# nvagus/mnexp

Measured on NVIDIA B200. Metric: lstur_train_impressions_per_sec, higher is better.
Workload: dtype f16

## Files before the change

### mnexp_b200/csrc/attn.cu

```cuda
#include <cuda_fp16.h>

#include <stdlib.h>

#include "common.cuh"

namespace lstur {

constexpr int ATT_THREADS = 128;
constexpr int ATT_MAX_L = 256;

__global__ void __launch_bounds__(ATT_THREADS)
attn_pool_fwd_kernel(int N, int L, int F, float* __restrict__ C, long long title_stride,
                     const int* __restrict__ tok, const float* __restrict__ ka, const float* __restrict__ ba,
                     float* __restrict__ p, long long ldp, float* __restrict__ a_out, float* __restrict__ w_out,
                     uint32_t drop_thr, float inv_keep, uint32_t seed) {
  __shared__ float sa[ATT_MAX_L], se[ATT_MAX_L];
  const int n = blockIdx.x, tid = threadIdx.x, warp = tid >> 5, lane = tid & 31;
  float* Cn = C + (long long)n * title_stride;
  const float bias = ba[0];
  for (int t = warp; t < L; t += ATT_THREADS / 32) {
    const int tk = tok[(long long)n * L + t];
    float dot = 0.f;
    int any = 0;
    const uint64_t base = ((uint64_t)n * L + t) * (uint64_t)F;
    for (int f = lane; f < F; f += 32) {
      float v = tk != 0 ? Cn[(long long)t * F + f] : 0.f;
      any |= (v != 0.f);
      if (drop_thr) v = (rng_u32(seed, base + f) >> 8) >= drop_thr ? v * inv_keep : 0.f;
      Cn[(long long)t * F + f] = v;
      dot = fmaf(v, ka[f], dot);
    }
    any = warp_or(any);
    dot = warp_sum(dot);
    if (lane == 0) {
      float a = tanhf(dot + bias);
      sa[t] = a;
      se[t] = any ? expf(a) : 0.f;
    }
  }
  __syncthreads();
  float S = 0.f;
  for (int t = 0; t < L; ++t) S += se[t];
  const float invS = 1.f / (S + 1e-7f);
  for (int t = tid; t < L; t += ATT_THREADS) {
    if (a_out) a_out[(long long)n * L + t] = sa[t];
    if (w_out) w_out[(long long)n * L + t] = se[t] * invS;
  }
  for (int f = tid; f < F; f += ATT_THREADS) {
    float acc = 0.f;
    for (int t = 0; t < L; ++t) acc = fmaf(se[t] * invS, Cn[(long long)t * F + f], acc);
    p[(long long)n * ldp + f] = acc;
  }
}

__device__ __forceinline__ float ldc(const float* p, long long i) { return p[i]; }
__device__ __forceinline__ float ldc(const __nv_bfloat16* p, long long i) { return __bfloat162float(p[i]); }
__device__ __forceinline__ float ldc(const __half* p, long long i) { return __half2float(p[i]); }

__device__ __forceinline__ void store_dpre_img(void* img, int out_mode, int ngh, int Fh, int n, int t, int f, float v) {
  const int h = f >= Fh ? 1 : 0, fl = f - h * Fh;
  const long long byte = (long long)n * ((long long)2 * ngh * 4096) + (long long)(h * ngh + (fl >> 6)) * 4096 + t * 128 +
                         ((((fl & 63) >> 3) ^ (t & 7)) << 4) + (fl & 7) * 2;
  if (out_mode == 2) *reinterpret_cast<__half*>((char*)img + byte) = __float2half_rn(fminf(fmaxf(v, -65504.f), 65504.f));
  else *reinterpret_cast<__nv_bfloat16*>((char*)img + byte) = __float2bfloat16_rn(v);
}

template <int FPT, typename CT, int OUT>
__global__ void __launch_bounds__(ATT_THREADS)
attn_pool_bwd_kernel(int N, int L, int Lrows, int F, const CT* __restrict__ Cd, long long title_stride,
                     const float* __restrict__ a_in, const float* __restrict__ w_in, const float* __restrict__ dp,
                     long long lddp, const float* __restrict__ ka, float* __restrict__ dPre,
                     long long dpre_title_stride, float inv_keep, float* __restrict__ partials) {
  __shared__ float sdw[ATT_MAX_L], sdz[ATT_MAX_L], sw[ATT_MAX_L];
  const int tid = threadIdx.x, warp = tid >> 5, lane = tid & 31;
  float dka[FPT], dbc[FPT], dba = 0.f;
#pragma unroll
  for (int i = 0; i < FPT; ++i) dka[i] = dbc[i] = 0.f;
  for (int n = blockIdx.x; n < N; n += gridDim.x) {
    const CT* Cn = Cd + (long long)n * title_stride;
    const float* dpn = dp + (long long)n * lddp;
    float* dPn = dPre + (long long)n * dpre_title_stride;
    for (int t = warp; t < L; t += ATT_THREADS / 32) {
      float dot = 0.f;
      for (int f = lane; f < F; f += 32) dot = fmaf(ldc(Cn, (long long)t * F + f), dpn[f], dot);
      dot = warp_sum(dot);
      if (lane == 0) {
        sdw[t] = dot;
        sw[t] = w_in[(long long)n * L + t];
      }
    }
    __syncthreads();
    float q = 0.f;
    for (int t = 0; t < L; ++t) q = fmaf(sdw[t], sw[t], q);
    for (int t = tid; t < L; t += ATT_THREADS) {
      float a = a_in[(long long)n * L + t];
      sdz[t] = (sdw[t] - q) * sw[t] * (1.f - a * a);
    }
    __syncthreads();
#pragma unroll
    for (int i = 0; i < FPT; ++i) {
      int f = tid + i * ATT_THREADS;
      if (f < F) {
        const float dpf = dpn[f], kaf = ka[f];
        for (int t = 0; t < L; ++t) {
          float c = ldc(Cn, (long long)t * F + f);
          float g = fmaf(sw[t], dpf, sdz[t] * kaf);
          float dpre = c > 0.f ? g * inv_keep : 0.f;
          if (OUT == 0) dPn[(long long)t * F + f] = dpre;
          else store_dpre_img(dPre, OUT, ((F >> 1) + 63) >> 6, F >> 1, n, t, f, dpre);
          dka[i] = fmaf(sdz[t], c, dka[i]);
          dbc[i] += dpre;
        }
        for (int t = L; t < Lrows; ++t) {
          if (OUT == 0) dPn[(long long)t * F + f] = 0.f;
          else store_dpre_img(dPre, OUT, ((F >> 1) + 63) >> 6, F >> 1, n, t, f, 0.f);
        }
      }
    }
    if (tid == 0)
      for (int t = 0; t < L; ++t) dba += sdz[t];
    __syncthreads();
  }
  float* out = partials + (long long)blockIdx.x * (2 * F + 1);
#pragma unroll
  for (int i = 0; i < FPT; ++i) {
    int f = tid + i * ATT_THREADS;
    if (f < F) {
      out[f] = dka[i];
      out[F + f] = dbc[i];
    }
  }
  if (tid == 0) out[2 * F] = dba;
}

__global__ void colsum_stage1_kernel(long long rows, int cols, const float* __restrict__ in, long long ld,
                                     int rows_per_chunk, float* __restrict__ partial) {
  int c = blockIdx.x * blockDim.x + threadIdx.x;
  if (c >= cols) return;
  long long r0 = (long long)blockIdx.y * rows_per_chunk, r1 = min(rows, r0 + rows_per_chunk);
  float s0 = 0.f, s1 = 0.f, s2 = 0.f, s3 = 0.f;
  long long r = r0;
  for (; r + 3 < r1; r += 4) {
    s0 += in[r * ld + c];
    s1 += in[(r + 1) * ld + c];
    s2 += in[(r + 2) * ld + c];
    s3 += in[(r + 3) * ld + c];
  }
  for (; r < r1; ++r) s0 += in[r * ld + c];
  partial[(long long)blockIdx.y * cols + c] = (s0 + s1) + (s2 + s3);
}
__global__ void colsum_stage2_kernel(int chunks, int cols, const float* __restrict__ partial, float* __restrict__ out,
                                     int accumulate) {
  __shared__ float sm[8][32];
  const int lane = threadIdx.x & 31, part = threadIdx.x >> 5;
  const int c = blockIdx.x * 32 + lane;
  float s = 0.f;
  if (c < cols)
    for (int k = part; k < chunks; k += 8) s += partial[(long long)k * cols + c];
  sm[part][lane] = s;
  __syncthreads();
  if (part != 0 || c >= cols) return;
  float t = 0.f;
#pragma unroll
  for (int q = 0; q < 8; ++q) t += sm[q][lane];
  out[c] = accumulate ? out[c] + t : t;
}

template <typename CT>
__device__ __forceinline__ void unpack8(const uint4& u, float* v);
template <>
__device__ __forceinline__ void unpack8<__half>(const uint4& u, float* v) {
  const __half2* h = reinterpret_cast<const __half2*>(&u);
#pragma unroll
  for (int i = 0; i < 4; ++i) { float2 f = __half22float2(h[i]); v[2 * i] = f.x; v[2 * i + 1] = f.y; }
}
template <>
__device__ __forceinline__ void unpack8<__nv_bfloat16>(const uint4& u, float* v) {
  const __nv_bfloat162* h = reinterpret_cast<const __nv_bfloat162*>(&u);
#pragma unroll
  for (int i = 0; i < 4; ++i) { float2 f = __bfloat1622float2(h[i]); v[2 * i] = f.x; v[2 * i + 1] = f.y; }
}
template <typename CT>
__device__ __forceinline__ uint4 pack8(const float* v);
template <>
__device__ __forceinline__ uint4 pack8<__half>(const float* v) {
  uint4 u;
  __half2* h = reinterpret_cast<__half2*>(&u);
#pragma unroll
  for (int i = 0; i < 4; ++i) {
    uint32_t w;
    asm("cvt.rn.satfinite.f16x2.f32 %0, %1, %2;" : "=r"(w) : "f"(v[2 * i + 1]), "f"(v[2 * i]));
    reinterpret_cast<uint32_t*>(&u)[i] = w;
  }
  (void)h;
  return u;
}
template <>
__device__ __forceinline__ uint4 pack8<__nv_bfloat16>(const float* v) {
  uint4 u;
  __nv_bfloat162* h = reinterpret_cast<__nv_bfloat162*>(&u);
#pragma unroll
  for (int i = 0; i < 4; ++i) h[i] = __floats2bfloat162_rn(v[2 * i], v[2 * i + 1]);
  return u;
}

constexpr int IMG_THREADS = 256;
template <typename CT, int SLOT>
__global__ void __launch_bounds__(IMG_THREADS)
attn_bwd_img_kernel(int N, int L, int F, const CT* __restrict__ Cd, const float* __restrict__ a_in,
                    const float* __restrict__ w_in, const float* __restrict__ dp, long long lddp,
                    const float* __restrict__ ka, uint8_t* __restrict__ img, float inv_keep, float img_scale,
                    float* __restrict__ partials, int nbuf, const int* __restrict__ n_dev,
                    const int* __restrict__ title_idx) {
  if (n_dev) N = min(N, __ldg(n_dev));
  extern __shared__ __align__(16) uint8_t att_smem[];
  const int nchunk = F >> 3;
  const size_t buf_bytes = (size_t)SLOT * nchunk * 16;
  float* sdp = reinterpret_cast<float*>(att_smem + nbuf * buf_bytes);
  float* ska = sdp + F;
  float* sred = reinterpret_cast<float*>(att_smem);
  __shared__ float sdw[SLOT], sdz[SLOT], sw[SLOT];
  __shared__ __align__(8) unsigned long long s_bar[2];
  const int tid = threadIdx.x, warp = tid >> 5, lane = tid & 31;
  const int c = tid & 63, tg = tid >> 6;
  const bool c_ok = c < nchunk;
  const int Fh = F >> 1, ngh = (Fh + 63) >> 6;
  constexpr int GROUP_BYTES = SLOT * 128;
  const long long blk_bytes = (long long)2 * ngh * GROUP_BYTES;
  const int pad_pieces = ((((Fh + 31) >> 5) << 5) - Fh) >> 3;
  const uint32_t title_bytes = (uint32_t)L * F * sizeof(CT);
  const uint32_t bar0 = (uint32_t)__cvta_generic_to_shared(&s_bar[0]);
  const uint32_t buf0 = (uint32_t)__cvta_generic_to_shared(att_smem);
  auto fetch_title = [&](int n, int b) {
    asm volatile("mbarrier.arrive.expect_tx.shared::cta.b64 _, [%0], %1;" ::"r"(bar0 + 8 * b), "r"(title_bytes) : "memory");
    asm volatile("cp.async.bulk.shared::cluster.global.mbarrier::complete_tx::bytes [%0], [%1], %2, [%3];" ::"r"(
                     buf0 + (uint32_t)(b * buf_bytes)),
                 "l"(Cd + (long long)n * L * F), "r"(title_bytes), "r"(bar0 + 8 * b)
                 : "memory");
  };
  if (tid == 0) {
    asm volatile("mbarrier.init.shared::cta.b64 [%0], 1;" ::"r"(bar0) : "memory");
    asm volatile("mbarrier.init.shared::cta.b64 [%0], 1;" ::"r"(bar0 + 8) : "memory");
    asm volatile("fence.mbarrier_init.release.cluster;" ::: "memory");
  }
  for (int f = tid; f < F; f += IMG_THREADS) ska[f] = ka[f];
  __syncthreads();
  float dka[8], dbc[8], dba = 0.f;
#pragma unroll
  for (int i = 0; i < 8; ++i) dka[i] = dbc[i] = 0.f;
  constexpr int DPR = 2;
  float ndp[DPR], nw = 0.f, na = 0.f;
  auto prefetch_small = [&](int n) {
    const int no = (title_idx && n < N) ? __ldg(title_idx + n) : n;
#pragma unroll
    for (int i = 0; i < DPR; ++i) {
      const int f = tid + i * IMG_THREADS;
      ndp[i] = (n < N && f < F) ? dp[(long long)no * lddp + f] : 0.f;
    }
    nw = (n < N && tid < L) ? w_in[(long long)n * L + tid] : 0.f;
    na = (n < N && tid < L) ? a_in[(long long)n * L + tid] : 0.f;
  };
  if (blockIdx.x < N) {
    if (tid == 0) fetch_title(blockIdx.x, 0);
    prefetch_small(blockIdx.x);
  }
  uint32_t phase[2] = {0, 0};
  int it = 0;
  for (int n = blockIdx.x; n < N; n += gridDim.x, ++it) {
    const int b = nbuf == 2 ? (it & 1) : 0;
    const uint4* sC = reinterpret_cast<const uint4*>(att_smem + b * buf_bytes);
    __syncthreads();
    const int n_next = n + gridDim.x;
    if (nbuf == 2) {
      if (tid == 0 && n_next < N) fetch_title(n_next, b ^ 1);
    } else if (it > 0) {
      if (tid == 0) fetch_title(n, 0);
    }
#pragma unroll
    for (int i = 0; i < DPR; ++i) {
      const int f = tid + i * IMG_THREADS;
      if (f < F) sdp[f] = ndp[i];
    }
    if (tid < L) sw[tid] = nw;
    const float a_cur = na;
    prefetch_small(n_next);
    {
      uint32_t done = 0;
      while (!done) {
        asm volatile(
            "{\n\t.reg .pred p;\n\t"
            "mbarrier.try_wait.parity.shared::cta.b64 p, [%1], %2;\n\t"
            "selp.u32 %0, 1, 0, p;\n\t}"
            : "=r"(done)
            : "r"(bar0 + 8 * b), "r"(phase[b])
            : "memory");
      }
      phase[b] ^= 1;
    }
    __syncthreads();
    {
      float dpa[2][8];
#pragma unroll
      for (int k = 0; k < 2; ++k) {
        const int cc = lane + 32 * k;
        const float4 lo = cc < nchunk ? *reinterpret_cast<const float4*>(sdp + cc * 8) : make_float4(0.f, 0.f, 0.f, 0.f);
        const float4 hi = cc < nchunk ? *reinterpret_cast<const float4*>(sdp + cc * 8 + 4) : make_float4(0.f, 0.f, 0.f, 0.f);
        dpa[k][0] = lo.x; dpa[k][1] = lo.y; dpa[k][2] = lo.z; dpa[k][3] = lo.w;
        dpa[k][4] = hi.x; dpa[k][5] = hi.y; dpa[k][6] = hi.z; dpa[k][7] = hi.w;
      }
#pragma unroll
      for (int tt = 0; tt < SLOT / 8; ++tt) {
// ... 282 lines not shown
```

### mnexp_b200/csrc/gather.cu

```cuda
#include "common.cuh"

namespace lstur {

__global__ void token_gather_kernel(int N, int L, int n_docs, const int* __restrict__ doc_tokens,
                                    const int* __restrict__ doc_ids, int* __restrict__ tokens) {
  int warp = (blockIdx.x * blockDim.x + threadIdx.x) >> 5, lane = threadIdx.x & 31;
  if (warp >= N) return;
  int d = doc_ids[warp];
  d = (d < 0 || d >= n_docs) ? 0 : d;
  const int* src = doc_tokens + (long long)d * L;
  int* dst = tokens + (long long)warp * L;
  for (int l = lane; l < L; l += 32) dst[l] = __ldg(src + l);
}

__global__ void embed_gather_pad_kernel(int N, int L, int E, int V, int KS, const float* __restrict__ word_emb,
                                        const int* __restrict__ tok, float* __restrict__ Xp, uint32_t drop_thr,
                                        float inv_keep, uint32_t seed, int Ep) {
  long long row = ((long long)blockIdx.x * blockDim.x + threadIdx.x) >> 5;
  int lane = threadIdx.x & 31;
  const int Lp = L + KS - 1;
  if (row >= (long long)N * Lp) return;
  int n = (int)(row / Lp), t = (int)(row % Lp) - (KS - 1) / 2;
  float* dst = Xp + row * E;
  if (t < 0 || t >= L) {
    for (int e = lane; e < E; e += 32) dst[e] = 0.f;
    return;
  }
  int id = tok[(long long)n * L + t];
  id = (id < 0 || id >= V) ? 0 : id;
  const float* src = word_emb + (long long)id * E;
  const uint64_t base = ((uint64_t)n * L + t) * (uint64_t)E;
  if (Ep > 0) {
    const uint64_t pbase = ((uint64_t)n * L + t) * (uint64_t)Ep;
    for (int e = lane; e < E; e += 32) {
      float v = __ldg(src + e);
      uint32_t h = rng_u32(seed, (pbase + e) >> 1);
      uint32_t h16 = (e & 1) ? (h >> 16) : (h & 0xffffu);
      dst[e] = h16 >= drop_thr ? v * inv_keep : 0.f;
    }
    return;
  }
  if ((E & 3) == 0) {
    for (int e = lane * 4; e < E; e += 128) {
      float4 v = __ldg((const float4*)(src + e));
      if (drop_thr) {
        v.x = (rng_u32(seed, base + e + 0) >> 8) >= drop_thr ? v.x * inv_keep : 0.f;
        v.y = (rng_u32(seed, base + e + 1) >> 8) >= drop_thr ? v.y * inv_keep : 0.f;
        v.z = (rng_u32(seed, base + e + 2) >> 8) >= drop_thr ? v.z * inv_keep : 0.f;
        v.w = (rng_u32(seed, base + e + 3) >> 8) >= drop_thr ? v.w * inv_keep : 0.f;
      }
      *(float4*)(dst + e) = v;
    }
  } else {
    for (int e = lane; e < E; e += 32) {
      float v = __ldg(src + e);
      if (drop_thr) v = (rng_u32(seed, base + e) >> 8) >= drop_thr ? v * inv_keep : 0.f;
      dst[e] = v;
    }
  }
}

__global__ void hist_mask_apply_kernel(int rows, int L, int D, const int* __restrict__ tok, float* __restrict__ H,
                                       long long ldh, float* __restrict__ hm_out, float* __restrict__ gm_out) {
  int warp = (blockIdx.x * blockDim.x + threadIdx.x) >> 5, lane = threadIdx.x & 31;
  if (warp >= rows) return;
  int nz = 1;
  if (tok) {
    nz = 0;
    for (int l = lane; l < L; l += 32) nz |= (tok[(long long)warp * L + l] != 0);
    nz = warp_or(nz);
  }
  float* h = H + (long long)warp * ldh;
  int any = 0;
  for (int d = lane; d < D; d += 32) {
    float v = nz ? h[d] : 0.f;
    h[d] = v;
    any |= (v != 0.f);
  }
  any = warp_or(any);
  if (lane == 0) {
    if (hm_out) hm_out[warp] = (tok ? nz : any) ? 1.f : 0.f;
    gm_out[warp] = any ? 1.f : 0.f;
  }
}

__global__ void row_gather_kernel(int B, int D, int n_rows, const float* __restrict__ table,
                                  const int* __restrict__ ids, const float* __restrict__ scale,
                                  float* __restrict__ out, long long ldo) {
  int warp = (blockIdx.x * blockDim.x + threadIdx.x) >> 5, lane = threadIdx.x & 31;
  if (warp >= B) return;
  int id = ids[warp];
  id = (id < 0 || id >= n_rows) ? 0 : id;
  float s = scale ? scale[warp] : 1.f;
  for (int d = lane; d < D; d += 32) out[(long long)warp * ldo + d] = __ldg(table + (long long)id * D + d) * s;
}


__global__ void vert_concat_kernel(int n, int D, int col0, int dv, int ds, int n_docs, int n_vert, int n_sub,
                                   const int* __restrict__ doc_ids, const int* __restrict__ doc_vert,
                                   const int* __restrict__ doc_subvert, const float* __restrict__ vert_emb,
                                   const float* __restrict__ subvert_emb, float* __restrict__ docv,
                                   int* __restrict__ tv, int* __restrict__ ts) {
  int warp = (blockIdx.x * blockDim.x + threadIdx.x) >> 5, lane = threadIdx.x & 31;
  if (warp >= n) return;
  int d = warp;
  if (doc_ids) {
    d = doc_ids[warp];
    d = (d < 0 || d >= n_docs) ? 0 : d;
  }
  int v = dv ? doc_vert[d] : 0, sv = ds ? doc_subvert[d] : 0;
  v = (v < 0 || v >= n_vert) ? 0 : v;
  sv = (sv < 0 || sv >= n_sub) ? 0 : sv;
  float* row = docv + (long long)warp * D + col0;
  for (int j = lane; j < dv; j += 32) row[j] = vert_emb[(long long)v * dv + j];
  for (int j = lane; j < ds; j += 32) row[dv + j] = subvert_emb[(long long)sv * ds + j];
  if (lane == 0) {
    if (tv) tv[warp] = v;
    if (ts) ts[warp] = sv;
  }
}

constexpr int STG_CHUNKS = 64;
__global__ void small_table_grad1_kernel(int n, int D, int col0, int dim, const int* __restrict__ ids,
                                         const float* __restrict__ dd, float* __restrict__ partial) {
  const int r = blockIdx.x, k = blockIdx.y, n_rows = gridDim.x;
  const int per = (n + STG_CHUNKS - 1) / STG_CHUNKS;
  const int beg = k * per, end = min(n, beg + per);
  float acc = 0.f;
  const int j = threadIdx.x;
  for (int i = beg; i < end; ++i)
    if (ids[i] == r && j < dim) acc += dd[(long long)i * D + col0 + j];
  if (j < dim) partial[((long long)k * n_rows + r) * dim + j] = acc;
}
__global__ void small_table_grad2_kernel(int n_rows, int dim, const float* __restrict__ partial, float* __restrict__ out) {
  const int i = blockIdx.x * blockDim.x + threadIdx.x;
  if (i >= n_rows * dim) return;
  float acc = 0.f;
  for (int k = 0; k < STG_CHUNKS; ++k) acc += partial[(long long)k * n_rows * dim + i];
  out[i] = acc;
}
__global__ void scale_rows_kernel(int B, int D, const float* __restrict__ scale, float* __restrict__ x, long long ld) {
  const long long i = (long long)blockIdx.x * blockDim.x + threadIdx.x;
  if (i >= (long long)B * D) return;
  const int b = (int)(i / D), d = (int)(i % D);
  x[(long long)b * ld + d] *= scale[b];
}


__global__ void assemble_batch_kernel(int B, int W, int K, const int* __restrict__ sample_click, const int* __restrict__ idx,
                                      const int* __restrict__ click_user, const int* __restrict__ stream_off,
                                      const int* __restrict__ stream_docs, const int* __restrict__ neg_off,
                                      const int* __restrict__ neg_docs, uint32_t seed, int* __restrict__ user_out,
                                      int* __restrict__ hist_out, int* __restrict__ cand_out) {
  const int T = W + 1 + K;
  const long long i = (long long)blockIdx.x * blockDim.x + threadIdx.x;
  if (i >= (long long)B * T) return;
  const int b = (int)(i / T), e = (int)(i % T);
  const int c = sample_click[idx[b]];
  const int u = click_user[c];
  const int off = stream_off[u];
  if (e < W) {
    const int j = c - W + e;
    hist_out[(long long)b * W + e] = j >= off ? stream_docs[j] : 0;
    if (e == 0) user_out[b] = u;
  } else if (e == W) {
    cand_out[(long long)b * (1 + K)] = stream_docs[c];
  } else {
    const int k = e - W - 1;
    const int n0 = neg_off[c], n = neg_off[c + 1] - n0;
    const uint32_t r = rng_u32(seed, (uint64_t)b * K + k);
    cand_out[(long long)b * (1 + K) + 1 + k] = n > 0 ? neg_docs[n0 + (int)(r % (uint32_t)n)] : 0;
  }
}

__global__ void title_live_kernel(int N, int L, const int* __restrict__ tok, int* __restrict__ flags) {
  int warp = (int)(((long long)blockIdx.x * blockDim.x + threadIdx.x) >> 5), lane = threadIdx.x & 31;
  if (warp >= N) return;
  int nz = 0;
  for (int l = lane; l < L; l += 32) nz |= (tok[(long long)warp * L + l] != 0);
  nz = warp_or(nz);
  if (lane == 0) flags[warp] = nz ? 1 : 0;
}
__global__ void __launch_bounds__(1024) title_rank_kernel(int N, const int* __restrict__ flags, int* __restrict__ local_rank,
                                                          int* __restrict__ block_tot) {
  __shared__ int wsum[32];
  const int n = blockIdx.x * 1024 + threadIdx.x, lane = threadIdx.x & 31, warp = threadIdx.x >> 5;
  const int f = (n < N && flags[n]) ? 1 : 0;
  const unsigned bal = __ballot_sync(0xffffffffu, f);
  if (lane == 0) wsum[warp] = __popc(bal);
  __syncthreads();
  if (warp == 0) {
    int v = wsum[lane];
#pragma unroll
    for (int o = 1; o < 32; o <<= 1) {
      const int u = __shfl_up_sync(0xffffffffu, v, o);
      if (lane >= o) v += u;
    }
    wsum[lane] = v;
  }
  __syncthreads();
  if (n < N) local_rank[n] = (warp ? wsum[warp - 1] : 0) + __popc(bal & ((1u << lane) - 1u));
  if (threadIdx.x == 0) block_tot[blockIdx.x] = wsum[31];
}
__global__ void title_compact_kernel(int N, int L, const int* __restrict__ tok, const int* __restrict__ flags,
                                     const int* __restrict__ local_rank, const int* __restrict__ block_tot, int n_blocks,
                                     int* __restrict__ live_idx, int* __restrict__ n_live, int* __restrict__ tok_c) {
  int warp = (int)(((long long)blockIdx.x * blockDim.x + threadIdx.x) >> 5), lane = threadIdx.x & 31;
  if (warp >= N) return;
  const int blk = warp >> 10;
  int before = 0;
  for (int b = lane; b < n_blocks; b += 32) before += (b < blk || warp == N - 1) ? block_tot[b] : 0;
  before = __reduce_add_sync(0xffffffffu, before);
  if (warp == N - 1) {
    if (lane == 0) *n_live = before;
    before = 0;
    for (int b = lane; b < blk; b += 32) before += block_tot[b];
    before = __reduce_add_sync(0xffffffffu, before);
  }
  if (!flags[warp]) return;
  const int ci = before + local_rank[warp];
  if (lane == 0) live_idx[ci] = warp;
  for (int l = lane; l < L; l += 32) tok_c[(long long)ci * L + l] = tok[(long long)warp * L + l];
}

__global__ void mask_live_kernel(int N, const int* __restrict__ v, int* __restrict__ flags) {
  const int n = blockIdx.x * blockDim.x + threadIdx.x;
  if (n < N) flags[n] = v[n] != 0 ? 1 : 0;
}
__global__ void __launch_bounds__(1024) mask_compact_kernel(int N, const int* __restrict__ v, const int* __restrict__ flags,
                                                            const int* __restrict__ local_rank,
// ... 163 lines not shown
```

### mnexp_b200/csrc/gemm_tc.cu

```cuda
#include <stdlib.h>

#include "tc_common.cuh"

namespace lstur {
namespace tc {

constexpr int G_KBLK = 64;
constexpr int G_STAGES = 4;
constexpr int G_A_BYTES = TILE_M * 128;
constexpr int G_B_BYTES = 256 * 128;
constexpr int G_STAGE_BYTES = G_A_BYTES + G_B_BYTES;
constexpr int G_STAGE_BYTES_S3 = 2 * (G_A_BYTES + G_B_BYTES);
constexpr int G_THREADS = 416;
constexpr int G_PRODUCERS = 256;

struct GemmParams {
  int M, N, K;
  const float* A; long long lda;
  const float* B; long long ldb;
  float* C; long long ldc;
  const float* bias;
  int flags, ntile, k_per_split, vec_ok;
  int tiles_m, tiles_n, splits;
  float* partial;
// ... 167 lines not shown
              const uint64_t ad = TA ? make_desc_mn128(a_addr + kk * 2048, 8192) : make_desc_k128(a_addr + kk * 32);
              const uint64_t bd = TB ? make_desc_k128(b_addr + kk * 32) : make_desc_mn128(b_addr + kk * 2048, 8192);
              umma_bf16(tacc, ad, bd, idesc, accum);
              accum = 1;
              if (SPLIT) {
                const uint64_t al = TA ? make_desc_mn128(a_addr + LO_OFF + kk * 2048, 8192) : make_desc_k128(a_addr + LO_OFF + kk * 32);
                const uint64_t bl = TB ? make_desc_k128(b_addr + LO_OFF + kk * 32) : make_desc_mn128(b_addr + LO_OFF + kk * 2048, 8192);
                umma_bf16(tacc, al, bd, idesc, 1);
                umma_bf16(tacc, ad, bl, idesc, 1);
              }
            }
            umma_commit(bar_empty + 8 * s);
          }
          accum = 1;
          __syncwarp();
          if (++s == STAGES) { s = 0; ph ^= 1; }
        }
        if (leader) umma_commit(bar_t_full + 8 * acc);
        __syncwarp();
        pht[acc] ^= 1;
        acc ^= 1;
      }
    }
  } else if (warp >= 1 && warp < 9) {
    const int pt = threadIdx.x - 32;
    int s = 0;
    uint32_t ph = 0;
    constexpr int BATCH = 6;
    for (int t = blockIdx.x; t < n_tiles; t += gridDim.x) {
      const Tile x = tile_of(t);
      const int m0 = x.m0, n0 = x.n0, nt = x.nt, kend = x.kend;
      const int bgroups = (x.nmma + 63) >> 6;
      const bool img = p.bimg != nullptr;
      const int nb_pieces = img ? 0 : (TB ? x.nmma * 8 : bgroups * 512);
      const uint32_t b_tile_bytes = (uint32_t)(TB ? x.nmma * 128 : bgroups * 8192);
      int arow[4];
#pragma unroll
      for (int idx = 0; idx < 4; ++idx) {
        const int r = m0 + ((pt + idx * G_PRODUCERS) >> 3);
        arow[idx] = r < Meff ? (p.midx ? __ldg(p.midx + r) : r) : p.M;
      }
      for (int kb = 0; kb < x.nkb; ++kb) {
        const int k0 = x.kbeg + kb * G_KBLK;
        const uint32_t a_addr = smem_base + s * STAGE_BYTES, b_addr = a_addr + G_A_BYTES;
        auto piece_load = [&](int idx, float* v) {
          if (idx < 4) {
            const int i = pt + idx * G_PRODUCERS, c = i & 7, r = i >> 3;
            if (!TA) load_raw(p.A, p.lda, arow[idx], p.M, k0 + 8 * c, kend, p.vec_ok, v);
            else load_raw(p.A, p.lda, k0 + (r & 63), kend, m0 + (r >> 6) * 64 + 8 * c, p.M, p.vec_ok, v);
          } else {
            const int i = pt + (idx - 4) * G_PRODUCERS, c = i & 7, r = i >> 3;
            if (i < nb_pieces) {
              if (TB) load_raw(p.B, p.ldb, n0 + r, n0 + nt, k0 + 8 * c, kend, p.vec_ok, v);
              else load_raw(p.B, p.ldb, k0 + (r & 63), kend, n0 + (r >> 6) * 64 + 8 * c, n0 + nt, p.vec_ok, v);
            }
          }
        };
        auto piece_store = [&](int idx, const float* v) {
          uint4 lo;
          if (idx < 4) {
            const int i = pt + idx * G_PRODUCERS, c = i & 7, r = i >> 3;
            const uint4 hi = cvt_piece<SPLIT>(v, lo);
            const uint32_t off = !TA ? (uint32_t)(r * 128 + ((c ^ (r & 7)) << 4))
                                     : (uint32_t)((r >> 6) * 8192 + (r & 63) * 128 + ((c ^ (r & 7)) << 4));
            sts128(a_addr + off, hi);
            if (SPLIT) sts128(a_addr + LO_OFF + off, lo);
          } else {
            const int i = pt + (idx - 4) * G_PRODUCERS, c = i & 7, r = i >> 3;
            if (i < nb_pieces) {
              const uint4 hi = cvt_piece<SPLIT>(v, lo);
              const uint32_t off = TB ? (uint32_t)(r * 128 + ((c ^ (r & 7)) << 4))
                                      : (uint32_t)((r >> 6) * 8192 + (r & 63) * 128 + ((c ^ (r & 7)) << 4));
              sts128(b_addr + off, hi);
              if (SPLIT) sts128(b_addr + LO_OFF + off, lo);
            }
          }
        };
        float v[BATCH][8];
#pragma unroll
        for (int j = 0; j < BATCH; ++j) piece_load(j, v[j]);
        if (lane == 0) mbar_wait(bar_empty + 8 * s, ph ^ 1, 22);
        __syncwarp();
        if (img && pt == 0) {
          const uint8_t* src = p.bimg + ((size_t)(n0 / p.ntile) * p.nkb_total + (size_t)(k0 / G_KBLK)) * (SPLIT ? 2 : 1) * G_BIMG_TILE;
          mbar_expect_tx(bar_full + 8 * s, b_tile_bytes * (SPLIT ? 2u : 1u));
          bulk_g2s(b_addr, src, b_tile_bytes, bar_full + 8 * s);
          if (SPLIT) bulk_g2s(b_addr + LO_OFF, src + G_BIMG_TILE, b_tile_bytes, bar_full + 8 * s);
        }
#pragma unroll
        for (int j = 0; j < BATCH; ++j) piece_store(j, v[j]);
        if (nb_pieces > (BATCH - 4) * G_PRODUCERS) {
#pragma unroll
          for (int j = 0; j < BATCH; ++j) piece_load(BATCH + j, v[j]);
#pragma unroll
          for (int j = 0; j < BATCH; ++j) piece_store(BATCH + j, v[j]);
        }
        fence_proxy_async();
        __syncwarp();
        if (lane == 0) mbar_arrive(bar_full + 8 * s);
        if (++s == STAGES) { s = 0; ph ^= 1; }
      }
    }
  } else if (warp >= 9) {
    const int q = warp & 3;
    int acc = 0;
    uint32_t pht[2] = {0, 0};
    const bool split = p.splits > 1;
    for (int t = blockIdx.x; t < n_tiles; t += gridDim.x) {
      const Tile x = tile_of(t);
      mbar_wait(bar_t_full + 8 * acc, pht[acc], 23);
      pht[acc] ^= 1;
      tc_fence_after();
      float* cbase = split ? p.partial + (long long)x.z * p.M * p.N : p.C;
      const long long ldo = split ? (long long)p.N : p.ldc;
      const bool vec_st = (ldo % 4 == 0) && ((((uintptr_t)cbase) & 15) == 0) && ((x.n0 & 3) == 0);
      int orow[8];
      if (p.midx) {
#pragma unroll
        for (int i = 0; i < 8; ++i) {
          const int rr = x.m0 + q * 32 + (lane >> 3) + 4 * i;
          orow[i] = rr < Meff ? __ldg(p.midx + rr) : -1;
        }
      }
      for (int c0 = 0; c0 < x.nmma; c0 += 32) {
        uint32_t r[32];
        const uint32_t taddr = tmem_base + acc * 256 + ((uint32_t)(q * 32) << 16) + (uint32_t)c0;
        if (x.nmma - c0 >= 32) { TMEM_LD_32(taddr, r); } else { TMEM_LD_16(taddr, r); }
        tmem_ld_wait();
        const int ncols = min(32, x.nt - c0);
        if (ncols > 0)
          gemm_epi_store(s_epi + (warp - 9) * (G_EPI_WARP_BYTES / 4), lane, r, x.nkb > 0, cbase, ldo, x.m0 + q * 32, Meff,
                         x.n0 + c0, ncols, p.bias, p.flags, !split, vec_st, p.midx ? orow : nullptr);
      }
      tc_fence_before();
      __syncwarp();
      if (lane == 0) mbar_arrive(bar_t_empty + 8 * acc);
      acc ^= 1;
    }
  }
  __syncthreads();
  if (warp == 0) {
    asm volatile("tcgen05.dealloc.cta_group::1.sync.aligned.b32 %0, %1;" ::"r"(tmem_base), "r"(512) : "memory");
  }
}

template <bool TB, bool SPLIT>
__global__ void gemm_pack_b_kernel(int N, int K, const float* __restrict__ B, long long ldb, int ntile, int vec_ok,
                                   uint8_t* __restrict__ img) {
  const int kb = blockIdx.x, tn = blockIdx.y, nkb_total = gridDim.x;
  const int n0 = tn * ntile, nt = min(ntile, N - n0), nmma = (nt + 15) & ~15, bgroups = (nmma + 63) >> 6;
  const int k0 = kb * G_KBLK;
  const int pieces = TB ? nmma * 8 : bgroups * 512;
  uint8_t* dst = img + ((size_t)tn * nkb_total + kb) * (SPLIT ? 2 : 1) * G_BIMG_TILE;
  for (int i = threadIdx.x; i < pieces; i += blockDim.x) {
    const int c = i & 7, r = i >> 3;
    float v[8];
    if (TB) load_raw(B, ldb, n0 + r, n0 + nt, k0 + 8 * c, K, vec_ok != 0, v);
    else load_raw(B, ldb, k0 + (r & 63), K, n0 + (r >> 6) * 64 + 8 * c, n0 + nt, vec_ok != 0, v);
    uint4 lo;
    const uint4 hi = cvt_piece<SPLIT>(v, lo);
    const uint32_t off = TB ? (uint32_t)(r * 128 + ((c ^ (r & 7)) << 4))
                            : (uint32_t)((r >> 6) * 8192 + (r & 63) * 128 + ((c ^ (r & 7)) << 4));
    *reinterpret_cast<uint4*>(dst + off) = hi;
    if (SPLIT) *reinterpret_cast<uint4*>(dst + G_BIMG_TILE + off) = lo;
  }
}

constexpr int GA_NT = 128;
constexpr int GA_RAW_A = TILE_M * G_KBLK * 4;
constexpr int GA_RAW_B = GA_NT * G_KBLK * 4;
constexpr int GA_RAW_STAGE = GA_RAW_A + GA_RAW_B;
constexpr int GA_F16_A = TILE_M * 128;
constexpr int GA_F16_B = GA_NT * 128;
constexpr int GA_F16_STAGE = GA_F16_A + GA_F16_B;

__device__ __forceinline__ void cp_async16(uint32_t dst, const void* src, bool valid) {
  const int sz = valid ? 16 : 0;
  asm volatile("cp.async.cg.shared.global [%0], [%1], 16, %2;" ::"r"(dst), "l"(src), "r"(sz) : "memory");
}
__device__ __forceinline__ void lds8(uint32_t addr, float* v) {
  float4 a, b;
  asm volatile("ld.shared.v4.f32 {%0,%1,%2,%3}, [%4];" : "=f"(a.x), "=f"(a.y), "=f"(a.z), "=f"(a.w) : "r"(addr));
  asm volatile("ld.shared.v4.f32 {%0,%1,%2,%3}, [%4];" : "=f"(b.x), "=f"(b.y), "=f"(b.z), "=f"(b.w) : "r"(addr + 16));
  v[0] = a.x; v[1] = a.y; v[2] = a.z; v[3] = a.w; v[4] = b.x; v[5] = b.y; v[6] = b.z; v[7] = b.w;
}

template <bool TA, bool TB, bool SPLIT>
__global__ void __launch_bounds__(G_THREADS, 1) gemm_tc_async_kernel(const GemmParams p) {
  constexpr int FST = SPLIT ? 1 : 2;
  constexpr int F16_STAGE = SPLIT ? 2 * GA_F16_STAGE : GA_F16_STAGE;
  constexpr int LO_OFF = GA_F16_STAGE;
  extern __shared__ __align__(1024) uint8_t smem_raw[];
  const uint32_t smem_base = (smem_u32(smem_raw) + 1023u) & ~1023u;
  uint8_t* smem_gen = smem_raw + (smem_base - smem_u32(smem_raw));
  const uint32_t f16_base = smem_base, raw_base = smem_base + FST * F16_STAGE;
  const uint32_t misc_base = raw_base + 2 * GA_RAW_STAGE;
  uint8_t* misc_gen = smem_gen + (misc_base - smem_base);
  const uint32_t bar_full = misc_base, bar_empty = misc_base + 64, bar_t_full = misc_base + 128, bar_t_empty = misc_base + 144;
  uint32_t* tmem_ptr_smem = (uint32_t*)(misc_gen + 160);
  float* s_epi = (float*)(misc_gen + 256);
  const int warp = threadIdx.x >> 5, lane = threadIdx.x & 31;
  const int n_tiles = p.tiles_m * p.tiles_n * p.splits;

  const int Keff = p.kcount ? min(__ldg(p.kcount), p.K) : p.K;
  const int kps = p.kcount ? max(G_KBLK, ((Keff + p.splits - 1) / p.splits + G_KBLK - 1) / G_KBLK * G_KBLK) : p.k_per_split;
  struct Tile { int m0, n0, nt, nmma, z, kbeg, kend, nkb; };
  auto tile_of = [&](int t) {
    Tile x;
    const int tn = t % p.tiles_n, tm = (t / p.tiles_n) % p.tiles_m;
    x.z = t / (p.tiles_n * p.tiles_m);
    x.m0 = tm * TILE_M;
    x.n0 = tn * p.ntile;
    x.nt = min(p.ntile, p.N - x.n0);
    x.nmma = (x.nt + 15) & ~15;
    x.kbeg = x.z * kps;
    x.kend = min(Keff, x.kbeg + kps);
    x.nkb = x.kend > x.kbeg ? (x.kend - x.kbeg + G_KBLK - 1) / G_KBLK : 0;
    return x;
  };

  if (threadIdx.x == 0) {
    for (int s = 0; s < FST; ++s) {
      mbar_init(bar_full + 8 * s, G_PRODUCERS / 32);
      mbar_init(bar_empty + 8 * s, 1);
    }
    for (int a = 0; a < 2; ++a) {
      mbar_init(bar_t_full + 8 * a, 1);
      mbar_init(bar_t_empty + 8 * a, 4);
    }
    fence_barrier_init();
  }
  if (warp == 0) {
    asm volatile("tcgen05.alloc.cta_group::1.sync.aligned.shared::cta.b32 [%0], %1;" ::"r"(smem_u32(tmem_ptr_smem)), "r"(256)
                 : "memory");
    asm volatile("tcgen05.relinquish_alloc_permit.cta_group::1.sync.aligned;" ::: "memory");
  }
  tc_fence_before();
  __syncthreads();
  tc_fence_after();
  const uint32_t tmem_base = *tmem_ptr_smem;

  if (warp == 0) {
    {
      const bool leader = elect_one();
      int s = 0, acc = 0;
      uint32_t ph = 0, pht[2] = {0, 0};
      for (int t = blockIdx.x; t < n_tiles; t += gridDim.x) {
        const Tile x = tile_of(t);
        const uint32_t idesc = make_idesc(TILE_M, x.nmma, true) | (TA ? (1u << 15) : 0u) | (!TB ? (1u << 16) : 0u);
        mbar_wait(bar_t_empty + 8 * acc, pht[acc] ^ 1, 24);
        tc_fence_after();
        const uint32_t tacc = tmem_base + acc * 128;
        uint32_t accum = 0;
        for (int kb = 0; kb < x.nkb; ++kb) {
          mbar_wait(bar_full + 8 * s, ph, 21);
          tc_fence_after();
          const uint32_t a_addr = f16_base + s * F16_STAGE, b_addr = a_addr + GA_F16_A;
          if (leader) {
#pragma unroll
            for (int kk = 0; kk < G_KBLK / 16; ++kk) {
              const uint64_t ad = TA ? make_desc_mn128(a_addr + kk * 2048, 8192) : make_desc_k128(a_addr + kk * 32);
              const uint64_t bd = TB ? make_desc_k128(b_addr + kk * 32) : make_desc_mn128(b_addr + kk * 2048, 8192);
              umma_bf16(tacc, ad, bd, idesc, accum);
              accum = 1;
              if (SPLIT) {
                const uint64_t al = TA ? make_desc_mn128(a_addr + LO_OFF + kk * 2048, 8192) : make_desc_k128(a_addr + LO_OFF + kk * 32);
                const uint64_t bl = TB ? make_desc_k128(b_addr + LO_OFF + kk * 32) : make_desc_mn128(b_addr + LO_OFF + kk * 2048, 8192);
                umma_bf16(tacc, al, bd, idesc, 1);
                umma_bf16(tacc, ad, bl, idesc, 1);
              }
            }
            umma_commit(bar_empty + 8 * s);
          }
          accum = 1;
          __syncwarp();
          if (++s == FST) { s = 0; ph ^= 1; }
        }
        if (leader) umma_commit(bar_t_full + 8 * acc);
        __syncwarp();
        pht[acc] ^= 1;
        acc ^= 1;
      }
    }
  } else if (warp >= 1 && warp < 9) {
    const int pt = threadIdx.x - 32;
    struct Iter { int t, kb; Tile x; };
    auto first = [&]() {
      Iter it;
      it.t = blockIdx.x; it.kb = 0;
      while (it.t < n_tiles && (it.x = tile_of(it.t)).nkb == 0) it.t += gridDim.x;
      return it;
    };
    auto advance = [&](Iter& it) {
      if (it.t >= n_tiles) return;
      if (++it.kb < it.x.nkb) return;
      it.kb = 0;
      it.t += gridDim.x;
      while (it.t < n_tiles && (it.x = tile_of(it.t)).nkb == 0) it.t += gridDim.x;
    };
    int krows[8];
    auto fetch_rows = [&](const Iter& it) {
      if (!p.kidx || it.t >= n_tiles) return;
      const int k0 = it.x.kbeg + it.kb * G_KBLK;
#pragma unroll
      for (int i = 0; i < 8; ++i) {
        const int kr = (pt >> 5) + 8 * i;
        krows[i] = (k0 + kr < it.x.kend) ? __ldg(p.kidx + k0 + kr) : 0;
// ... 100 lines not shown
      const long long ldo = split ? (long long)p.N : p.ldc;
      const bool vec_st = (ldo % 4 == 0) && ((((uintptr_t)cbase) & 15) == 0) && ((x.n0 & 3) == 0);
      for (int c0 = 0; c0 < x.nmma; c0 += 32) {
        uint32_t r[32];
        const uint32_t taddr = tmem_base + acc * 128 + ((uint32_t)(q * 32) << 16) + (uint32_t)c0;
        if (x.nmma - c0 >= 32) { TMEM_LD_32(taddr, r); } else { TMEM_LD_16(taddr, r); }
        tmem_ld_wait();
        const int ncols = min(32, x.nt - c0);
        if (ncols > 0)
          gemm_epi_store(s_epi + (warp - 9) * (G_EPI_WARP_BYTES / 4), lane, r, x.nkb > 0, cbase, ldo, x.m0 + q * 32, p.M,
                         x.n0 + c0, ncols, p.bias, p.flags, !split, vec_st);
      }
      tc_fence_before();
      __syncwarp();
      if (lane == 0) mbar_arrive(bar_t_empty + 8 * acc);
      acc ^= 1;
    }
  }
  __syncthreads();
  if (warp == 0) {
    asm volatile("tcgen05.dealloc.cta_group::1.sync.aligned.b32 %0, %1;" ::"r"(tmem_base), "r"(256) : "memory");
  }
}

__global__ void gemm_tc_splitk_reduce_kernel(int M, int N, int splits, const float* __restrict__ partial,
                                             float* __restrict__ C, long long ldc, const float* __restrict__ bias,
                                             int flags) {
  long long i = (long long)blockIdx.x * blockDim.x + threadIdx.x;
  if (i >= (long long)M * N) return;
  int gm = (int)(i / N), gn = (int)(i % N);
  float v = 0.f;
  for (int s = 0; s < splits; ++s) v += partial[(long long)s * M * N + i];
  if (bias) v += bias[gn];
  if (flags & LSTUR_GEMM_ACCUM) v += C[(long long)gm * ldc + gn];
  if (flags & LSTUR_GEMM_RELU) v = fmaxf(v, 0.f);
  C[(long long)gm * ldc + gn] = v;
}

}
}

using namespace lstur;

static bool g_gemm_async = true;
static void gemm_tc_tiling(int M, int N, int K, int* ntile, int* splits, int max_nt = 256) {
  int nparts = (N + max_nt - 1) / max_nt;
  int nt = ((N + nparts - 1) / nparts + 15) & ~15;
  if (nt > max_nt) nt = max_nt;
  long long tiles = (long long)((M + tc::TILE_M - 1) / tc::TILE_M) * ((N + nt - 1) / nt);
  int sp = 1;
  if (tiles < 148 && K >= 2048) {
    sp = (int)(148 / tiles);
    int maxs = K / 512;
    if (sp > maxs) sp = maxs;
    if (sp < 1) sp = 1;
  }
  *ntile = nt;
  *splits = sp;
}

extern "C" size_t lstur_gemm_tc_workspace_bytes(int M, int N, int K) {
  int nt, sp, sp2;
  gemm_tc_tiling(M, N, K, &nt, &sp);
  gemm_tc_tiling(M, N, K, &nt, &sp2, tc::GA_NT);
  if (sp2 > sp) sp = sp2;
  size_t b = sp > 1 ? (size_t)sp * M * N * sizeof(float) : 0;
  gemm_tc_tiling(M, N, K, &nt, &sp);
  const size_t img = (size_t)((N + nt - 1) / nt) * ((K + tc::G_KBLK - 1) / tc::G_KBLK) * 2 * tc::G_BIMG_TILE;
  if (M >= 1024 && img > b) b = img;
  return b;
}

static int gemm_tc_impl(int transA, int transB, int M, int N, int K, const float* A, long long lda, const float* B,
                        long long ldb, float* C, long long ldc, const float* bias, int flags, void* workspace,
                        size_t workspace_bytes, const int* kidx, const int* kcount, cudaStream_t stream,
                        const int* midx = nullptr, const int* mcount = nullptr);

extern "C" int lstur_gemm_tc(int transA, int transB, int M, int N, int K, const float* A, long long lda, const float* B,
                             long long ldb, float* C, long long ldc, const float* bias, int flags, void* workspace,
                             size_t workspace_bytes, cudaStream_t stream) {
  return gemm_tc_impl(transA, transB, M, N, K, A, lda, B, ldb, C, ldc, bias, flags, workspace, workspace_bytes, nullptr, nullptr,
                      stream);
}

extern "C" int lstur_gemm_tc_tn_rows(int M, int N, int K, const float* A, long long lda, const float* B, long long ldb, float* C,
                                     long long ldc, const int* k_rows, const int* k_count, void* workspace,
                                     size_t workspace_bytes, cudaStream_t stream) {
  return gemm_tc_impl(1, 0, M, N, K, A, lda, B, ldb, C, ldc, nullptr, 0, workspace, workspace_bytes, k_rows, k_count, stream);
}

extern "C" int lstur_gemm_tc_mrows(int transB, int M, int N, int K, const float* A, long long lda, const float* B, long long ldb,
                                   float* C, long long ldc, const float* bias, int flags, const int* m_rows, const int* m_count,
                                   void* workspace, size_t workspace_bytes, cudaStream_t stream) {
  return gemm_tc_impl(0, transB, M, N, K, A, lda, B, ldb, C, ldc, bias, flags, workspace, workspace_bytes, nullptr, nullptr, stream,
                      m_rows, m_count);
}

static int gemm_tc_impl(int transA, int transB, int M, int N, int K, const float* A, long long lda, const float* B,
                        long long ldb, float* C, long long ldc, const float* bias, int flags, void* workspace,
                        size_t workspace_bytes, const int* kidx, const int* kcount, cudaStream_t stream,
                        const int* midx, const int* mcount) {
  LSTUR_REQUIRE(M >= 0 && N >= 0 && K >= 0, "lstur_gemm_tc");
  if (M == 0 || N == 0) return LSTUR_OK;
  tc::GemmParams p;
  int splits;
  static bool env_read = false;
  if (!env_read) {
    const char* e = getenv("LSTUR_GEMM_ASYNC");
    if (e && atoi(e) == 0) g_gemm_async = false;
    env_read = true;
  }
  const bool rows16 = (lda % 4 == 0) && (ldb % 4 == 0) && ((((uintptr_t)A) & 15) == 0) && ((((uintptr_t)B) & 15) == 0) &&
                      ((transA ? M : K) % 4 == 0) && ((transB ? K : N) % 4 == 0);
  const bool use_async = g_gemm_async && rows16 && K > 0 && transA;
  gemm_tc_tiling(M, N, K, &p.ntile, &splits, use_async ? tc::GA_NT : 256);
  size_t need = splits > 1 ? (size_t)splits * M * N * sizeof(float) : 0;
  if (need > workspace_bytes || (need && !workspace)) splits = 1;
  int kps = ((K + splits - 1) / splits + tc::G_KBLK - 1) / tc::G_KBLK * tc::G_KBLK;
  if (kps == 0) kps = tc::G_KBLK;
  splits = K > 0 ? (K + kps - 1) / kps : 1;
  p.M = M; p.N = N; p.K = K; p.A = A; p.lda = lda; p.B = B; p.ldb = ldb; p.C = C; p.ldc = ldc; p.bias = bias;
  p.flags = flags; p.k_per_split = kps; p.partial = (float*)workspace;
  p.bimg = nullptr; p.nkb_total = (K + tc::G_KBLK - 1) / tc::G_KBLK;
  p.kidx = use_async ? kidx : nullptr;
  p.kcount = use_async ? kcount : nullptr;
  p.midx = nullptr; p.mcount = nullptr;
  p.vec_ok = (lda % 4 == 0) && (ldb % 4 == 0) && ((((uintptr_t)A) & 15) == 0) && ((((uintptr_t)B) & 15) == 0);
  const bool split3 = (flags & LSTUR_GEMM_PRECISE) != 0;
  size_t smem = 1024 + (split3 ? (size_t)2 * tc::G_STAGE_BYTES_S3 : (size_t)tc::G_STAGES * tc::G_STAGE_BYTES) + 256 +
                4 * tc::G_EPI_WARP_BYTES;
  static bool attr = false;
  if (!attr) {
    const int big = 1024 + 2 * tc::G_STAGE_BYTES_S3 + 256 + 4 * tc::G_EPI_WARP_BYTES;
    cudaError_t e = cudaSuccess;
#define SETATTR(TA_, TB_, S_) \
  if (e == cudaSuccess) e = cudaFuncSetAttribute(tc::gemm_tc_kernel<TA_, TB_, S_>, cudaFuncAttributeMaxDynamicSharedMemorySize, big)
    SETATTR(false, false, false); SETATTR(true, false, false); SETATTR(false, true, false); SETATTR(true, true, false);
    SETATTR(false, false, true); SETATTR(true, false, true); SETATTR(false, true, true); SETATTR(true, true, true);
#undef SETATTR
    if (e != cudaSuccess) {
      set_error("lstur_gemm_tc: cannot opt in to %d B of shared memory: %s", big, cudaGetErrorString(e));
      return LSTUR_ERR_CUDA;
    }
    attr = true;
  }
  p.tiles_n = (N + p.ntile - 1) / p.ntile;
  p.tiles_m = (M + tc::TILE_M - 1) / tc::TILE_M;
  p.splits = splits;
  if (midx && mcount && !use_async && !transA && splits == 1) { p.midx = midx; p.mcount = mcount; }
  static int img_mode = -1;
  if (img_mode < 0) { const char* e = getenv("LSTUR_GEMM_BIMG"); img_mode = (e && atoi(e) == 0) ? 0 : 1; }
  const size_t img_bytes = (size_t)p.tiles_n * p.nkb_total * (split3 ? 2 : 1) * tc::G_BIMG_TILE;
  if (img_mode && !use_async && !transA && splits == 1 && M >= 1024 && K > 0 && workspace && img_bytes <= workspace_bytes) {
    dim3 pg((unsigned)p.nkb_total, (unsigned)p.tiles_n);
    uint8_t* img = (uint8_t*)workspace;
    if (transB) {
      if (split3) tc::gemm_pack_b_kernel<true, true><<<pg, 256, 0, stream>>>(N, K, B, ldb, p.ntile, p.vec_ok, img);
      else tc::gemm_pack_b_kernel<true, false><<<pg, 256, 0, stream>>>(N, K, B, ldb, p.ntile, p.vec_ok, img);
    } else {
      if (split3) tc::gemm_pack_b_kernel<false, true><<<pg, 256, 0, stream>>>(N, K, B, ldb, p.ntile, p.vec_ok, img);
      else tc::gemm_pack_b_kernel<false, false><<<pg, 256, 0, stream>>>(N, K, B, ldb, p.ntile, p.vec_ok, img);
    }
    LSTUR_CHECK_LAUNCH("lstur_gemm_tc(pack B)");
    p.bimg = img;
  }
  const long long n_tiles = (long long)p.tiles_m * p.tiles_n * splits;
  int sms = 148;
  cudaDeviceGetAttribute(&sms, cudaDevAttrMultiProcessorCount, 0);
  dim3 grid((unsigned)(n_tiles < sms ? n_tiles : sms));
  const size_t smem_async = 1024 + (size_t)2 * tc::GA_F16_STAGE + (size_t)2 * tc::GA_RAW_STAGE + 256 + 4 * tc::G_EPI_WARP_BYTES;
  static bool attr_async = false;
  if (use_async && !attr_async) {
    cudaError_t e = cudaSuccess;
#define SETATTR(TA_, TB_, S_) \
  if (e == cudaSuccess) e = cudaFuncSetAttribute(tc::gemm_tc_async_kernel<TA_, TB_, S_>, cudaFuncAttributeMaxDynamicSharedMemorySize, (int)smem_async)
    SETATTR(false, false, false); SETATTR(true, false, false); SETATTR(false, true, false); SETATTR(true, true, false);
    SETATTR(false, false, true); SETATTR(true, false, true); SETATTR(false, true, true); SETATTR(true, true, true);
#undef SETATTR
    if (e != cudaSuccess) {
      set_error("lstur_gemm_tc: cannot opt in to %zu B of shared memory: %s", smem_async, cudaGetErrorString(e));
      return LSTUR_ERR_CUDA;
    }
    attr_async = true;
  }
#define LAUNCH(TA_, TB_)                                                                                \
  do {                                                                                                  \
    if (use_async) {                                                                                    \
      if (split3) tc::gemm_tc_async_kernel<TA_, TB_, true><<<grid, tc::G_THREADS, smem_async, stream>>>(p);  \
      else tc::gemm_tc_async_kernel<TA_, TB_, false><<<grid, tc::G_THREADS, smem_async, stream>>>(p);        \
    } else {                                                                                            \
      if (split3) tc::gemm_tc_kernel<TA_, TB_, true><<<grid, tc::G_THREADS, smem, stream>>>(p);         \
      else tc::gemm_tc_kernel<TA_, TB_, false><<<grid, tc::G_THREADS, smem, stream>>>(p);               \
    }                                                                                                   \
  } while (0)
  if (!transA && !transB) LAUNCH(false, false);
  else if (transA && !transB) LAUNCH(true, false);
  else if (!transA && transB) LAUNCH(false, true);
  else LAUNCH(true, true);
#undef LAUNCH
  LSTUR_CHECK_LAUNCH("lstur_gemm_tc");
  if (splits > 1) {
    long long n = (long long)M * N;
    tc::gemm_tc_splitk_reduce_kernel<<<cdiv(n, 256), 256, 0, stream>>>(M, N, splits, p.partial, C, ldc, bias, flags);
    LSTUR_CHECK_LAUNCH("lstur_gemm_tc(splitk_reduce)");
  }
  return LSTUR_OK;
}
```

Before: 344,600.

## Batch column-sum loads, skip redundant history rewrites, and widen B-pack grid

The column-sum kernels now issue 32 (stage 1) or 8 (stage 2) independent loads before accumulating, which raises memory-level parallelism. The history mask kernel no longer writes back rows that are kept unchanged. It only reads them to test for nonzeros, and writes zeros only for masked rows. The GEMM B-image pack kernel gains a z grid dimension so each tile's pieces are spread over more blocks. Costs are higher register pressure in the unrolled loops and extra small blocks in the pack launch.

```diff
diff --git a/mnexp_b200/csrc/attn.cu b/mnexp_b200/csrc/attn.cu
--- a/mnexp_b200/csrc/attn.cu
+++ b/mnexp_b200/csrc/attn.cu
@@ -140,6 +140,13 @@
   long long r0 = (long long)blockIdx.y * rows_per_chunk, r1 = min(rows, r0 + rows_per_chunk);
   float s0 = 0.f, s1 = 0.f, s2 = 0.f, s3 = 0.f;
   long long r = r0;
+  for (; r + 31 < r1; r += 32) {
+    float v[32];
+#pragma unroll
+    for (int i = 0; i < 32; ++i) v[i] = in[(r + i) * ld + c];
+#pragma unroll
+    for (int j = 0; j < 8; ++j) { s0 += v[4 * j]; s1 += v[4 * j + 1]; s2 += v[4 * j + 2]; s3 += v[4 * j + 3]; }
+  }
   for (; r + 3 < r1; r += 4) {
     s0 += in[r * ld + c];
     s1 += in[(r + 1) * ld + c];
@@ -155,8 +162,17 @@
   const int lane = threadIdx.x & 31, part = threadIdx.x >> 5;
   const int c = blockIdx.x * 32 + lane;
   float s = 0.f;
-  if (c < cols)
-    for (int k = part; k < chunks; k += 8) s += partial[(long long)k * cols + c];
+  if (c < cols) {
+    int k = part;
+    for (; k + 56 < chunks; k += 64) {
+      float v[8];
+#pragma unroll
+      for (int i = 0; i < 8; ++i) v[i] = partial[(long long)(k + 8 * i) * cols + c];
+#pragma unroll
+      for (int i = 0; i < 8; ++i) s += v[i];
+    }
+    for (; k < chunks; k += 8) s += partial[(long long)k * cols + c];
+  }
   sm[part][lane] = s;
   __syncthreads();
   if (part != 0 || c >= cols) return;
diff --git a/mnexp_b200/csrc/gather.cu b/mnexp_b200/csrc/gather.cu
--- a/mnexp_b200/csrc/gather.cu
+++ b/mnexp_b200/csrc/gather.cu
@@ -72,10 +72,14 @@
   }
   float* h = H + (long long)warp * ldh;
   int any = 0;
-  for (int d = lane; d < D; d += 32) {
-    float v = nz ? h[d] : 0.f;
-    h[d] = v;
-    any |= (v != 0.f);
+  if (nz) {
+    for (int d0 = lane; d0 < D; d0 += 256) {
+#pragma unroll
+      for (int i = 0; i < 8; ++i)
+        if (d0 + 32 * i < D) any |= (h[d0 + 32 * i] != 0.f);
+    }
+  } else {
+    for (int d = lane; d < D; d += 32) h[d] = 0.f;
   }
   any = warp_or(any);
   if (lane == 0) {
diff --git a/mnexp_b200/csrc/gemm_tc.cu b/mnexp_b200/csrc/gemm_tc.cu
--- a/mnexp_b200/csrc/gemm_tc.cu
+++ b/mnexp_b200/csrc/gemm_tc.cu
@@ -343,7 +343,7 @@
   const int k0 = kb * G_KBLK;
   const int pieces = TB ? nmma * 8 : bgroups * 512;
   uint8_t* dst = img + ((size_t)tn * nkb_total + kb) * (SPLIT ? 2 : 1) * G_BIMG_TILE;
-  for (int i = threadIdx.x; i < pieces; i += blockDim.x) {
+  for (int i = blockIdx.z * blockDim.x + threadIdx.x; i < pieces; i += gridDim.z * blockDim.x) {
     const int c = i & 7, r = i >> 3;
     float v[8];
     if (TB) load_raw(B, ldb, n0 + r, n0 + nt, k0 + 8 * c, K, vec_ok != 0, v);
@@ -750,7 +750,8 @@
   if (img_mode < 0) { const char* e = getenv("LSTUR_GEMM_BIMG"); img_mode = (e && atoi(e) == 0) ? 0 : 1; }
   const size_t img_bytes = (size_t)p.tiles_n * p.nkb_total * (split3 ? 2 : 1) * tc::G_BIMG_TILE;
   if (img_mode && !use_async && !transA && splits == 1 && M >= 1024 && K > 0 && workspace && img_bytes <= workspace_bytes) {
-    dim3 pg((unsigned)p.nkb_total, (unsigned)p.tiles_n);
+    const int nmma = (p.ntile + 15) & ~15, pieces = transB ? nmma * 8 : ((nmma + 63) >> 6) * 512;
+    dim3 pg((unsigned)p.nkb_total, (unsigned)p.tiles_n, (unsigned)cdiv(pieces, 256));
     uint8_t* img = (uint8_t*)workspace;
     if (transB) {
       if (split3) tc::gemm_pack_b_kernel<true, true><<<pg, 256, 0, stream>>>(N, K, B, ldb, p.ntile, p.vec_ok, img);
```

New measurement: 347,900 (median of 6 runs). No clear change (+1.0%).
